# Savasstion/FYPRayTracer

Hardware: AMD Instinct MI355X
Metric: Mrays/s at 1920x1080, 1 spp ReSTIR DI (ms/frame in ms_per_step) (higher is better)
Workload: dtype f32; 1 GPU; hall_1M_tris_256_lights_1920x1080_RESTIR_DI_1spp; triangles=999832, meshes=108, emissive_triangles=256, rays_per_frame=3932782, temporal_reuse=True, spatial_reuse=True, parallelism=row-bands x1

## Files before the change

### fypraytracer_amd/csrc/fyprt.hip

```cpp
#include <hip/hip_runtime.h>
#include <atomic>
#include <cmath>
#include <cstdio>
#include <cstring>
#include <functional>
#include <string>
#include <vector>
#include "rt_host.h"
#include <hipcub/hipcub.hpp>
#include "rt_lbvh.h"
#include "rt_refit.h"
#include "rt_materials.h"
#include "rt_paths.h"
#include "rt_query.h"
#include "rt_points.h"
#include "rt_boxes.h"
#include "rt_denoise.h"
#include "rt_temporal.h"
#include "rt_upscale.h"
#include "rt_probe.h"

using namespace rt;

#ifndef RT_DN_LDS_MAX_STEP
// ... 1459 lines not shown
    const uint32_t tilesX = (c->W + 15u) / 16u, tilesY = (rowEnd - rowBegin + 15u) / 16u;
    return dim3(c->tuning[K_TILE_ORDER] == 2 ? tilesX * ((tilesY + 7u) / 8u) * 8u : ((tilesX * tilesY + 7u) / 8u) * 8u);
}
static unsigned long long* frame_counters(const fyprt_context* c, int part) { return c->countRays ? c->rayCounter.p + 8 * part : nullptr; }
static int check_frame(fyprt_context* c, const fyprt_settings* s, int phase) {
    if (c->hostOnly) return c->fail(FYPRT_ESTATE, "host-only context (device -1) cannot render");
    if (!c->haveScene || !c->haveCamera || c->W == 0) return c->fail(FYPRT_ESTATE, "fyprt_render: resize, upload_scene and set_camera must precede render");
    if (c->dcam.W != c->W || c->dcam.H != c->H) return c->fail(FYPRT_ESTATE, "fyprt_render: camera viewport differs from the render size");
    const int tech = s->technique; const bool restir = tech == FYPRT_RESTIR_DI || tech == FYPRT_RESTIR_GI;
    if (tech < 0 || tech > 8) return c->fail(FYPRT_EINVAL, "fyprt_render: unknown technique");
    if (phase != 0 && !restir) return c->fail(FYPRT_EINVAL, "fyprt_render_part: only the ReSTIR techniques have two parts");
    if (phase == 2 && !c->part1Pending) return c->fail(FYPRT_ESTATE, "fyprt_render_part(2) without a preceding part 1");
    if (phase != 2 && c->part1Pending) return c->fail(FYPRT_ESTATE, "a frame's part 1 is pending: call fyprt_render_part(ctx, settings, 2) first");
    if ((tech == FYPRT_LIGHT_SOURCE_SAMPLING || tech == FYPRT_NEE) && (c->dsc.emissiveCount == 0 || c->dsc.ltTlasCount == 0))
        return c->fail(FYPRT_ENOLIGHT, "fyprt_render: technique needs emissive triangles and a light tree");
    if (tech == FYPRT_RESTIR_DI && c->dsc.emissiveCount == 0) return c->fail(FYPRT_ENOLIGHT, "fyprt_render: ReSTIR DI needs emissive triangles");
    if (restir && stripes_set(c)) return c->fail(FYPRT_ESTATE, "ReSTIR frames need contiguous rows: clear fyprt_set_row_stripes first");
    return FYPRT_OK;
}
static int begin_frame(FrameRun& f) {
    fyprt_context* c = f.c; DevFrame& fr = f.fr;
    HIPCHK(c, hipSetDevice(c->device));
    f.st = dev_settings(c, f.s);
    fr.accum = c->accum.p; fr.image = c->externalImage ? c->externalImage : c->image.p; fr.payload = c->payload.p; fr.depth = c->depth.p;
    fr.normalPrev = c->normalFlip ? c->normalB.p : c->normalA.p; fr.normalCur = c->normalFlip ? c->normalA.p : c->normalB.p;
    fr.di = c->di.p; fr.diPrev = c->diPrev.p; fr.gi = c->gi.p; fr.giPrev = c->giPrev.p; fr.giHot = c->giHot.p;
    fr.drec = c->drec.p; fr.dprevRead = c->dprevFlip ? c->dprevB.p : c->dprevA.p; fr.dprevWrite = c->dprevFlip ? c->dprevA.p : c->dprevB.p;
    fr.W = c->W; fr.H = c->H; fr.frameIndex = c->frameIndex; fr.rowBegin = c->rowBegin; fr.rowEnd = c->rowEnd;
    fr.stripeRows = 0; fr.stripeParts = 1; fr.stripePart = 0; f.striped = stripes_set(c);
    fr.histBegin = (f.tech == FYPRT_RESTIR_GI) ? c->histGI[0] : c->histDI[0]; fr.histEnd = (f.tech == FYPRT_RESTIR_GI) ? c->histGI[1] : c->histDI[1];
#ifdef RT_TOPCACHE
    const uint32_t topCount = (uint32_t)std::min<size_t>((size_t)std::max(0, c->tuning[K_TOP_NODES]), c->hostBvh.nodes.size());
#else
    const uint32_t topCount = 0u;
#endif
    const StackLds stack = stack_lds(c, topCount);
    f.sc = secondary_scene(c->dsc, (uint32_t)c->tuning[K_QUORUM_PRIMARY], frame_counters(c, 0));
    f.sc.stackBudget = stack.budget; f.sc.topCount = topCount; f.ldsBytes = stack.bytes;
    f.par = (int)(c->frameSerial & 1ull); f.wavefront = f.tech == FYPRT_RESTIR_DI && c->tuning[K_DI_WAVEFRONT] == 1;
    f.overlap = f.wavefront && c->tuning[K_PIPELINE] != 0 && !c->countRays && f.phase == 0;
    f.fs = f.overlap ? c->front : c->stream;
    f.split = f.overlap && c->tuning[K_DI_SPLIT] != 0 && !c->blockingCall;
    if (f.overlap) {
        HIPCHK(c, hipStreamWaitEvent(c->front, c->evDone[f.par], 0));
        if (!c->lastOverlapped) HIPCHK(c, hipStreamWaitEvent(c->front, c->evDone[f.par ^ 1], 0));
    }
    if (f.split) HIPCHK(c, hipStreamWaitEvent(c->prim, c->evTemp[f.par], 0));
    c->frameComplete = false;
    if (f.tech != FYPRT_RESTIR_DI) c->drop_kept_primary();
    fr.tileOrder = (uint32_t)c->tuning[K_TILE_ORDER]; fr.p1Mode = f.wavefront ? 1u : 0u;
    f.grid = tile_grid(c, c->rowBegin, c->rowEnd); f.ev = c->ring[c->frameSerial % fyprt_context::kRing];
    if (f.phase == 2) { f.ei = 2; return FYPRT_OK; }
    std::memcpy(c->framePV, c->camPV, 64);
    c->frameCam = c->dcam; c->frameSky = f.st.sky;
    if (c->countRays) HIPCHK(c, hipMemsetAsync(c->rayCounter.p, 0, 256, c->stream));
    if (c->frameIndex == 1) HIPCHK(c, hipMemsetAsync(c->accum.p, 0, c->accum.bytes(), c->stream));
    if (f.timed) HIPCHK(c, hipEventRecord(f.ev[f.ei++], f.split ? c->prim.h : f.fs));
    return FYPRT_OK;
}
static int run_frame_stage(FrameRun& f, const StageRun& r) {
    fyprt_context* c = f.c;
    const StageBufs wf{{c->wfRays[0].p, c->wfRays[1].p}, {c->wfHits[0].p, c->wfHits[1].p}, c->wfState.p, c->wfPixels.p, c->wfPixels2.p, frame_counters(c, 0)};
    return run_stage(c, r, wf, f.sc, c->dcam, f.fr, f.st, f.ldsBytes, c->blockingCall, &f.stageLaunches);
}
static int enqueue_path_frame(FrameRun& f) {
    fyprt_context* c = f.c; DevFrame& fr = f.fr; const int tech = f.tech;
    const PathShape p = path_shape(tech, f.st);
    dim3 pgrid = f.grid;
    if (f.striped) {
        fr.stripeRows = c->stripeRows; fr.stripeParts = c->stripeParts; fr.stripePart = c->stripePart;
        fr.rowBegin = 0; fr.rowEnd = stripe_row_count(c->H, c->stripeRows, c->stripeParts, c->stripePart);
        pgrid = tile_grid(c, fr.rowBegin, fr.rowEnd);
    }
    const size_t entries = (size_t)(fr.rowEnd - fr.rowBegin) * c->W;
    TRY(ensure_paths(c, entries, p.raysPer, p.stride, 3 * p.L));
    HIPCHK(c, hipMemsetAsync(c->wfCounters.p, 0, 3 * p.L * sizeof(uint32_t), c->stream));
    f.launches = 1;
    const bool fused = tech != FYPRT_NEE && (c->tuning[K_FUSED_FRAME] == 2 || (c->tuning[K_FUSED_FRAME] == 0 && c->hostBvh.tris.size() < 65536u));
    if (fused) {
        PathIO io{};
        io.fusedOwner = kNotFused; io.raysIn = c->wfRays[0].p; io.raysOut = c->wfRays[0].p; io.hitsIn = c->wfHits[0].p; io.state = c->wfState.p; io.stateStride = p.stride; io.raysPer = 1u;
        static void (*const kFused[2][6])(DevScene, DevCamera, DevFrame, DevSettings, PathIO, uint32_t) = {{k_path_fused<T_BRUTE, false>, k_path_fused<T_UNIFORM, false>, k_path_fused<T_COSINE, false>, k_path_fused<T_GGX, false>, k_path_fused<T_BRDF, false>, k_path_fused<T_LIGHT, false>},
                                                    {k_path_fused<T_BRUTE, true>, k_path_fused<T_UNIFORM, true>, k_path_fused<T_COSINE, true>, k_path_fused<T_GGX, true>, k_path_fused<T_BRDF, true>, k_path_fused<T_LIGHT, true>}};
        hipLaunchKernelGGL(kFused[c->countRays ? 1 : 0][tech], pgrid, dim3(kBlock), f.ldsBytes, c->stream, f.sc, c->dcam, fr, f.st, io, p.steps);
        return FYPRT_OK;
    }
    hipLaunchKernelGGL(c->countRays ? k_primary<true> : k_primary<false>, pgrid, dim3(kBlock), f.ldsBytes, c->stream, f.sc, c->dcam, fr, f.st, c->wfPixels.p, c->wfCounters.p);
    return run_frame_stage(f, path_stage(tech, p, c->wfPixels.p, c->wfPixels2.p, c->wfCounters.p, entries));
}
struct Part1Rows { uint32_t begin, end, extraRow; size_t pixels; dim3 grid; };
static Part1Rows part1_rows(const fyprt_context* c) {
    const uint32_t halo = (c->haloExchange || c->tuning[K_SKIP_HALO_PART1]) ? 0u : c->halo;
    const uint32_t b = (c->rowBegin > halo) ? c->rowBegin - halo : 0u, e = (c->rowEnd + halo < c->H) ? c->rowEnd + halo : c->H;
    const bool extra = halo > 0 && c->rowBegin < halo && e < c->H;
    return {b, e, extra ? c->H - 1u : 0xFFFFFFFFu, ((size_t)(e - b) + (extra ? 1u : 0u)) * c->W, tile_grid(c, b, extra ? e + 16u : e)};
}
static int enqueue_gi_frame(FrameRun& f) {
    fyprt_context* c = f.c; const Part1Rows p1 = part1_rows(c);
    const uint32_t steps1 = f.st.maxBounces, steps2 = f.st.useSpatial ? f.st.numNeighbors : 0u;
    const size_t L1 = (size_t)steps1 + 2, L2 = (size_t)steps2 + 2;
    TRY(ensure_paths(c, p1.pixels, 1, 5, 2 * L1 + 2 * L2));
    uint32_t* cnt1 = c->wfCounters.p; uint32_t* cnt2 = cnt1 + 2 * L1;
    if (f.phase != 2) {
        TRY(sync_restir_normals(c, f.tech, c->stream));
        HIPCHK(c, hipMemsetAsync(cnt1, 0, (2 * L1 + 2 * L2) * sizeof(uint32_t), c->stream));
        hipLaunchKernelGGL(c->countRays ? k_gi_primary<true> : k_gi_primary<false>, p1.grid, dim3(kBlock), f.ldsBytes, c->stream, f.sc, c->dcam, f.fr, f.st, p1.begin, p1.end, p1.extraRow, c->wfPixels.p, cnt1);
        TRY(run_frame_stage(f, StageRun{T_GI1, steps1, 1u, 5u, c->wfPixels.p, cnt1, cnt1 + L1, c->wfPixels2.p, cnt2, 0, nullptr, p1.pixels}));
        if (f.timed) HIPCHK(c, hipEventRecord(f.ev[f.ei++], c->stream));
        if (f.phase == 1) { f.part1Only = true; return c->hip(hipGetLastError(), "ReSTIR GI part 1"); }
    }
    const DevScene tsc = secondary_scene(f.sc, (uint32_t)c->tuning[K_QUORUM_SECONDARY], frame_counters(c, 1));
    if (c->tuning[K_GI2_MODE] == 2) {
        const int occ = c->gi2Occ.get(k_gi2_persistent<false>, f.ldsBytes, 3), perCU = c->tuning[K_WG_PER_CU] > 0 ? std::min(c->tuning[K_WG_PER_CU], occ) : occ;
        GI2Queue gq{c->wfPixels2.p, cnt2, cnt2 + L2 + 1};
        set_queue_params(c, gq, K_GI2_REFILL_LANES);
        hipLaunchKernelGGL(c->countRays ? k_gi2_persistent<true> : k_gi2_persistent<false>, dim3((uint32_t)(c->numCUs * perCU)), dim3(kBlock), f.ldsBytes, c->stream, tsc, c->dcam, f.fr, f.st, gq);
    } else if (c->tuning[K_GI2_MODE] == 1) {
        const uint32_t fg = (uint32_t)std::max<size_t>(1, std::min<size_t>((size_t)c->numCUs * 64u, (p1.pixels + kBlock - 1) / kBlock));
        hipLaunchKernelGGL(c->countRays ? k_gi2_fused<true> : k_gi2_fused<false>, dim3(fg), dim3(kBlock), f.ldsBytes, c->stream, tsc, c->dcam, f.fr, f.st, (const uint32_t*)c->wfPixels2.p, (const uint32_t*)cnt2);
    } else TRY(run_frame_stage(f, StageRun{T_GI2, steps2, 1u, 5u, c->wfPixels2.p, cnt2, cnt2 + L2, nullptr, nullptr, 1, nullptr, p1.pixels}));
    f.launches = 2; c->normalFlip = !c->normalFlip; c->histGI[0] = c->rowBegin; c->histGI[1] = c->rowEnd;
    return FYPRT_OK;
}
static int enqueue_di_wavefront_part2(FrameRun& f) {
    fyprt_context* c = f.c; const int par = f.par; const dim3 grid = f.grid; hipStream_t fs = f.fs;
    const dim3 block(kBlock);
    ShadowQueue q{};
    q.tasks = c->shadowTasks.p + (size_t)par * c->queueStride; q.rayless = q.tasks + c->queueStride; q.counters = c->queueCounters.p + 4 * par;
    set_queue_params(c, q, K_REFILL_LANES);
    const size_t sg = (size_t)par * c->sortGroups;
    q.sortMode = c->tuning[K_SORT_TASKS] ? 1u : 0u; q.numGroups = grid.x; q.counts = c->sortCounts.p + 2 * sg; q.bases = q.counts + c->sortGroups; q.keys = c->sortKeys.p + sg * 256u; q.hist = c->sortHist.p + sg * kSortBins;
    q.binOffset = c->sortOffset.p + sg * kSortBins; q.binTotal = c->sortTotal.p + (size_t)par * kSortBins; q.sorted = c->sortIndex.p + sg * 256u;
    HIPCHK(c, hipMemsetAsync(q.counters, 0, 16, fs));
    static void (*const kSetup[3])(DevScene, DevCamera, DevFrame, DevSettings, ShadowQueue) = {k_di_part2_setup<0>, k_di_part2_setup<1>, k_di_part2_setup<2>};
    hipLaunchKernelGGL(kSetup[c->tuning[K_SETUP_FETCH]], grid, block, 0, fs, f.sc, c->dcam, f.fr, f.st, q);
    if (q.sortMode) {
        hipLaunchKernelGGL(k_di_sort_scan, dim3(kSortBins), block, 0, fs, q);
        hipLaunchKernelGGL(k_di_sort_scatter, grid, block, 0, fs, q);
    }
    if (f.timed) HIPCHK(c, hipEventRecord(f.ev[f.ei++], fs));
    if (f.overlap) {
        HIPCHK(c, hipEventRecord(c->evFront[par], c->front));
        HIPCHK(c, hipStreamWaitEvent(c->stream, c->evFront[par], 0));
        if (f.timed) HIPCHK(c, hipEventRecord(f.ev[4], c->stream));
    }
    f.sc.rayCounter = frame_counters(c, 2);
    int perCU = c->tuning[K_WG_PER_CU];
    if (perCU <= 0) {
        perCU = c->traceOcc.get(k_di_part2_trace<false>, f.ldsBytes, 4);
        if (f.overlap && perCU > 4) perCU = 4;
    }
    const uint32_t traceGrid = std::max(8u, std::min((uint32_t)(c->numCUs * perCU), grid.x));
    hipLaunchKernelGGL(c->countRays ? k_di_part2_trace<true> : k_di_part2_trace<false>, dim3(traceGrid), block, f.ldsBytes, c->stream, f.sc, f.fr, q);
    f.launches = 3;
    return FYPRT_OK;
}
static bool kept_primary_usable(const fyprt_context* c, const Part1Rows& p1) {
    const fyprt_context::KeptPrimary& k = c->kept; const DevCamera& d = c->dcam;
    return k.valid && !c->countRays && c->tuning[K_KEEP_PRIMARY] != 0 && k.begin == p1.begin && k.end == p1.end && k.extraRow == p1.extraRow && k.rowBegin == c->rowBegin && k.rowEnd == c->rowEnd && k.W == d.W && k.H == d.H &&
           !std::memcmp(&k.invProj, &d.invProj, sizeof d.invProj) && !std::memcmp(&k.invView, &d.invView, sizeof d.invView) && !std::memcmp(&k.position, &d.position, sizeof d.position);
}
static int establish_kept_primary(fyprt_context* c, const Part1Rows& p1, hipStream_t writer) {
    fyprt_context::KeptPrimary& k = c->kept; const DevCamera& d = c->dcam;
    k.valid = true; k.begin = p1.begin; k.end = p1.end; k.extraRow = p1.extraRow; k.rowBegin = c->rowBegin; k.rowEnd = c->rowEnd; k.invProj = d.invProj; k.invView = d.invView; k.position = d.position; k.W = d.W; k.H = d.H; k.writer = writer;
    HIPCHK(c, hipEventRecord(c->evPayload, writer));
    return FYPRT_OK;
}
static int enqueue_di_frame(FrameRun& f) {
    fyprt_context* c = f.c;
    if (f.phase != 2) {
        const Part1Rows p1 = part1_rows(c);
        const bool kept = kept_primary_usable(c, p1);
        if (kept) c->keptFrames++;
        if (f.split) {
            const size_t npx = (size_t)c->W * c->H;
            const DIStage sg{kept ? nullptr : c->stagePayload.p + (size_t)f.par * npx, c->stageRec.p + (size_t)f.par * npx};
            if (kept) {
                HIPCHK(c, hipStreamWaitEvent(c->prim, c->evPayload, 0));
                hipLaunchKernelGGL((k_di_part1_primary<false, true>), p1.grid, dim3(kBlock), 0, c->prim, f.sc, c->dcam, f.fr, f.st, p1.begin, p1.end, p1.extraRow, sg);
            } else hipLaunchKernelGGL((k_di_part1_primary<false, false>), p1.grid, dim3(kBlock), f.ldsBytes, c->prim, f.sc, c->dcam, f.fr, f.st, p1.begin, p1.end, p1.extraRow, sg);
            if (f.timed) HIPCHK(c, hipEventRecord(f.ev[f.ei++], c->prim));
            HIPCHK(c, hipEventRecord(c->evPrim[f.par], c->prim));
            HIPCHK(c, hipStreamWaitEvent(c->front, c->evPrim[f.par], 0));
            TRY(sync_restir_normals(c, f.tech, f.fs));
            if (f.timed) HIPCHK(c, hipEventRecord(f.ev[5], c->front));
            if (kept && c->kept.writer != c->front.h) HIPCHK(c, hipStreamWaitEvent(c->front, c->evPayload, 0));
            hipLaunchKernelGGL(kept ? k_di_part1_temporal<true> : k_di_part1_temporal<false>, p1.grid, dim3(kBlock), 0, c->front, f.sc, c->dcam, f.fr, f.st, p1.begin, p1.end, p1.extraRow, sg);
            HIPCHK(c, hipEventRecord(c->evTemp[f.par], c->front));
            if (!kept) TRY(establish_kept_primary(c, p1, c->front));
        } else {
            TRY(sync_restir_normals(c, f.tech, f.fs));
            if (kept) {
                if (c->kept.writer != f.fs) HIPCHK(c, hipStreamWaitEvent(f.fs, c->evPayload, 0));
                hipLaunchKernelGGL((k_di_part1<false, true>), p1.grid, dim3(kBlock), 0, f.fs, f.sc, c->dcam, f.fr, f.st, p1.begin, p1.end, p1.extraRow);
            } else {
                for (int k = 0; k < 2; ++k) HIPCHK(c, hipStreamWaitEvent(f.fs, c->evPrim[k], 0));
                hipLaunchKernelGGL((c->countRays ? k_di_part1<true, false> : k_di_part1<false, false>), p1.grid, dim3(kBlock), f.ldsBytes, f.fs, f.sc, c->dcam, f.fr, f.st, p1.begin, p1.end, p1.extraRow);
                TRY(establish_kept_primary(c, p1, f.fs));
            }
            if (f.timed) HIPCHK(c, hipEventRecord(f.ev[f.ei++], f.fs));
        }
        if (f.phase == 1) { f.part1Only = true; return c->hip(hipGetLastError(), "ReSTIR DI part 1"); }
    }
    f.sc = secondary_scene(f.sc, (uint32_t)c->tuning[K_QUORUM_SECONDARY], frame_counters(c, 1)); f.launches = 2;
    if (f.wavefront) TRY(enqueue_di_wavefront_part2(f));
    else hipLaunchKernelGGL(c->countRays ? k_di_part2<true> : k_di_part2<false>, f.grid, dim3(kBlock), f.ldsBytes, c->stream, f.sc, c->dcam, f.fr, f.st);
    c->dprevFlip = !c->dprevFlip; c->histDI[0] = c->rowBegin; c->histDI[1] = c->rowEnd;
    return FYPRT_OK;
}
static int end_frame(FrameRun& f) {
    fyprt_context* c = f.c; const unsigned long long slot = c->frameSerial % fyprt_context::kRing;
    HIPCHK(c, hipGetLastError());
    c->part1Pending = false;
    if (f.timed) HIPCHK(c, hipEventRecord(f.ev[f.ei++], c->stream));
    HIPCHK(c, hipEventRecord(c->evDone[f.par], c->stream));
    c->lastOverlapped = f.overlap; c->lastLaunches = f.launches; c->lastTech = f.tech;
    if (f.tech == FYPRT_RESTIR_DI || f.tech == FYPRT_RESTIR_GI) c->lastRestir = f.tech;
    c->ringLaunches[slot] = f.timed ? f.launches : 0; c->ringSplit[slot] = f.split ? 2 : f.overlap ? 1 : 0;
    c->frameSerial++; c->frameComplete = true; c->lastFrameIndex = c->frameIndex;
    if (f.s->to_accumulate) c->frameIndex++; else c->frameIndex = 1;
    return FYPRT_OK;
}
static int enqueue_frame(fyprt_context* c, const fyprt_settings* s, bool timed, int phase = 0) {
    FrameRun f{}; f.c = c; f.s = s; f.tech = s->technique; f.phase = phase; f.timed = timed;
    int rc = check_frame(c, s, phase);
    if (rc == FYPRT_OK) rc = begin_frame(f);
    if (rc == FYPRT_OK) rc = f.tech == FYPRT_RESTIR_DI ? enqueue_di_frame(f) : f.tech == FYPRT_RESTIR_GI ? enqueue_gi_frame(f) : enqueue_path_frame(f);
    if (rc == FYPRT_OK) { if (f.part1Only) c->part1Pending = true; else rc = end_frame(f); }
    if (rc != FYPRT_OK && rc != FYPRT_ESTATE) c->part1Pending = false;
    return rc;
}
static hipError_t part_elapsed(fyprt_context* c, unsigned long long slot, int k, float* ms) {
    const int mode = c->ringSplit[slot], start = (mode && k == 2) ? 4 : (mode == 2 && k == 1) ? 5 : k;
    return hipEventElapsedTime(ms, c->ring[slot][start], c->ring[slot][k + 1]);
}

int fyprt_render(fyprt_context* c, const fyprt_settings* s, fyprt_frame_stats* stats) {
    if (!c || !s) return FYPRT_EINVAL;
    c->blockingCall = true;
    int rc = enqueue_frame(c, s, true);
    c->blockingCall = false;
    if (rc != FYPRT_OK) return rc;
    HIPCHK(c, sync_all(c));
    if (stats) {
        std::memset(stats, 0, sizeof *stats);
        stats->launches = (uint32_t)c->lastLaunches;
        float total = 0.0f;
        for (int k = 0; k < c->lastLaunches; ++k) {
            float ms = 0.0f; (void)part_elapsed(c, (c->frameSerial - 1ull) % fyprt_context::kRing, k, &ms);
            stats->kernel_ms_part[k] = ms; total += ms;
        }
        stats->kernel_ms = total;
        if (c->countRays) {
            unsigned long long r[32] = {0}; (void)hipMemcpy(r, c->rayCounter.p, 256, hipMemcpyDeviceToHost);
            for (int k = 0; k < 4; ++k) add_ray_stats(stats, k, r + 8 * k);
        }
    }
    return FYPRT_OK;
}

int fyprt_render_async(fyprt_context* c, const fyprt_settings* s) { if (!c || !s) return FYPRT_EINVAL; return enqueue_frame(c, s, true); }

int fyprt_frame_timings(fyprt_context* c, uint32_t frames_back, float* kernel_ms_part4, uint32_t* launches) {
    if (!c || !kernel_ms_part4) return FYPRT_EINVAL;
    if (frames_back >= (uint32_t)fyprt_context::kRing || frames_back >= c->frameSerial) return c->fail(FYPRT_EINVAL, "fyprt_frame_timings: frame no longer in the ring");
    const unsigned long long slot = (c->frameSerial - 1ull - frames_back) % fyprt_context::kRing;
    const int n = c->ringLaunches[slot];
    for (int k = 0; k < 4; ++k) kernel_ms_part4[k] = 0.0f;
    for (int k = 0; k < n && k < 4; ++k) {
        float ms = 0.0f;
        const hipError_t e = part_elapsed(c, slot, k, &ms);
        if (e != hipSuccess) return c->hip(e, "hipEventElapsedTime (synchronize the context first)");
        kernel_ms_part4[k] = ms;
    }
    if (launches) *launches = (uint32_t)n;
    return FYPRT_OK;
}
int fyprt_synchronize(fyprt_context* c) { if (!c) return FYPRT_EINVAL; if (c->hostOnly) return FYPRT_OK; HIPCHK(c, hipSetDevice(c->device)); HIPCHK(c, sync_all(c)); return FYPRT_OK; }

int fyprt_readback(fyprt_context* c, uint32_t* rgba8, float* accum4) {
    if (!c) return FYPRT_EINVAL;
    if (c->hostOnly || c->W == 0) return c->fail(FYPRT_ESTATE, "fyprt_readback before fyprt_resize");
    HIPCHK(c, hipSetDevice(c->device));
    HIPCHK(c, sync_all(c));
    const size_t off = (size_t)c->rowBegin * c->W, cnt = (size_t)(c->rowEnd - c->rowBegin) * c->W;
    const uint32_t* img = c->externalImage ? c->externalImage : c->image.p;
    if (rgba8) HIPCHK(c, hipMemcpy(rgba8 + off, img + off, cnt * 4, hipMemcpyDeviceToHost));
    if (accum4) HIPCHK(c, hipMemcpy(accum4 + off * 4, c->accum.p + off, cnt * 16, hipMemcpyDeviceToHost));
    return FYPRT_OK;
}

int fyprt_selftest_math(fyprt_context* c, uint64_t* mismatches3, uint32_t* first_bad3) {
    if (!c || !mismatches3) return FYPRT_EINVAL;
    if (c->hostOnly) return c->fail(FYPRT_ESTATE, "fyprt_selftest_math needs a device");
    HIPCHK(c, hipSetDevice(c->device)); HIPCHK(c, sync_all(c));
    DevBuf<unsigned long long> counts; DevBuf<uint32_t> first;
    HIPCHK(c, counts.alloc(3)); HIPCHK(c, first.alloc(3));
    hipError_t e = hipMemsetAsync(counts.p, 0, 24, c->stream);
    if (e == hipSuccess) e = hipMemsetAsync(first.p, 0xFF, 12, c->stream);
    for (int w = 0; w < 3 && e == hipSuccess; ++w) { hipLaunchKernelGGL(k_math_selftest, dim3((uint32_t)c->numCUs * 16u), dim3(256), 0, c->stream, w, counts.p, first.p); e = hipGetLastError(); }
    unsigned long long hc[3] = {0, 0, 0}; uint32_t hf[3] = {0, 0, 0};
    if (e == hipSuccess) e = hipMemcpyAsync(hc, counts.p, 24, hipMemcpyDeviceToHost, c->stream);
    if (e == hipSuccess) e = hipMemcpyAsync(hf, first.p, 12, hipMemcpyDeviceToHost, c->stream);
    if (e == hipSuccess) e = hipStreamSynchronize(c->stream);
    HIPCHK(c, e);
    for (int w = 0; w < 3; ++w) { mismatches3[w] = hc[w]; if (first_bad3) first_bad3[w] = hf[w]; }
// ... 843 lines not shown
```

### fypraytracer_amd/csrc/rt_wavefront.h

```cpp
#pragma once
#include "rt_kernels.h"

namespace rt {

struct ShadowQueue {
    float4* tasks; uint32_t* counters; uint32_t chunk, refillLanes, staticChunks, minChunk;
    float4* rayless;
    uint32_t sortMode, numGroups; uint32_t* counts; uint32_t* bases; uint8_t* keys; uint16_t* hist; uint32_t* binOffset; uint32_t* binTotal; uint32_t* sorted;
};
constexpr uint32_t kNoRayTask = 0xFFFFFFFFu;
constexpr uint32_t kSortBins = 64;
constexpr int kRefillLanes = 16;

constexpr int kSpecNeighbors = 5;
RT_DEV uint32_t neighbor_from_states(const DevCamera& cam, uint32_t W, uint32_t x, uint32_t y, uint32_t radius, uint32_t s1, uint32_t s2) {
    float ox = 2.0f * ((float)s1 * 0x1p-32f) - 1.0f, oy = 2.0f * ((float)s2 * 0x1p-32f) - 1.0f;
    ox = (float)(uint32_t)(x + (uint32_t)(int)(ox * (float)radius));
    oy = (float)(uint32_t)(y + (uint32_t)(int)(oy * (float)radius));
    ox = __builtin_fmaxf(0.0f, __builtin_fminf((float)cam.W - 1.0f, ox));
    oy = __builtin_fmaxf(0.0f, __builtin_fminf((float)cam.H - 1.0f, oy));
    return (uint32_t)ox + (uint32_t)oy * W;
}
RT_DEV uint32_t spatial_reuse_speculative(const DevCamera& cam, const DevFrame& fr, const DevSettings& st, uint32_t x, uint32_t y, const Payload& pp, uint32_t seed, DIRes& S, uint32_t& Z) {
    const uint32_t N = st.numNeighbors;
// ... 74 lines not shown
    bool live = false, noRay = false;
    f3 ro = splat3(0.0f), rd = splat3(0.0f), Lvis = splat3(0.0f), Lsky = splat3(0.0f); uint32_t ti = kNoRayTask, lightSlot = 0; float tLight = -1.0f;
    Payload pp; Mat hm;
    if (inside) {
        pp = fr.payload[i];
        if (pp.hitDistance < 0.0f) { noRay = true; Lvis = st.sky; }
        else {
            hm = load_mat(sc, tri_material(sc, pp.objectIndex));
            if (length(emission(hm)) > 0.0f) { noRay = true; Lvis = emission(hm); } else live = true;
        }
    }
    if (live) {
        uint32_t seed = i * (fr.frameIndex + 213u + st.randSeed);
        const DIRec own = load_rec(fr.drec + i);
        DIRes R = rec_reservoir(own);
        const f3 pd = ray_direction(cam, x, y);
        if (st.useSpatial) {
            uint32_t Z = 0; DIRes S = di_empty();
            { const float pdf = R.pdf; di_update(S, R.index, (pdf * R.W) * (float)R.M, R.M, pdf, seed); Z += pdf > 0.0f ? R.M : 0u; }
            if (SPECULATIVE && st.numNeighbors <= (uint32_t)kSpecNeighbors) seed = spatial_reuse_speculative(cam, fr, st, x, y, pp, seed, S, Z);
            else if (MODE == 2 && ww != 0u) for (uint32_t n = 0; n < st.numNeighbors; ++n) {
                const uint32_t ni = neighbor_index(cam, fr.W, x, y, st.radius, seed);
                const uint32_t nxp = ni % fr.W, nyp = ni / fr.W;
                float nd; f2 nn;
                if (nxp - wx0 < ww && nyp - wy0 < wh) { const uint32_t k = (nyp - wy0) * ww + (nxp - wx0); nd = s_win[k]; nn.x = s_win[kWinMax * kWinMax + k]; nn.y = s_win[2 * kWinMax * kWinMax + k]; }
                else { const float4 h = reinterpret_cast<const float4*>(fr.drec + ni)[0]; nd = h.x; nn.x = h.y; nn.y = h.z; }
                const float pdp = pp.hitDistance;
                if ((nd > 1.1f * pdp || nd < 0.9f * pdp) || (double)dot(nrm3(pp), oct_decode(nn)) < 0.906) continue;
                const DIRes N = rec_reservoir(load_rec(fr.drec + ni));
                const float pdf = N.pdf;
                di_update(S, N.index, (pdf * N.W) * (float)N.M, N.M, pdf, seed);
                Z += pdf > 0.0f ? N.M : 0u;
            }
            else for (uint32_t n = 0; n < st.numNeighbors; ++n) {
                const uint32_t ni = neighbor_index(cam, fr.W, x, y, st.radius, seed);
                const DIRec nb = load_rec(fr.drec + ni);
                const float nd = nb.hitDistance, pdp = pp.hitDistance;
                f2 nn; nn.x = nb.nx; nn.y = nb.ny;
                const DIRes N = rec_reservoir(nb);
                if ((nd > 1.1f * pdp || nd < 0.9f * pdp) || (double)dot(nrm3(pp), oct_decode(nn)) < 0.906) continue;
                const float pdf = N.pdf;
                di_update(S, N.index, (pdf * N.W) * (float)N.M, N.M, pdf, seed);
                Z += pdf > 0.0f ? N.M : 0u;
            }
            const float m = 1.0f / (float)Z;
            S.W = S.pdf > 0.0f ? (1.0f / S.pdf) * (m * S.wSum) : 0.0f;
            R = S;
        }
        lightSlot = R.index;
        const float4* LR = sc.lightRecs + (size_t)R.index * 3;
        const float4 l0 = LR[0], l1 = LR[1], l2 = LR[2];
        ti = (uint32_t)__float_as_int(l1.w);
        const TriGeom g = load_tri(sc, ti);
        const f3 ep = tri_random_point(g, seed);
        f3 dir = ep - pos3(pp);
        const float dist = length(pos3(pp) - ep);
        dir = dir / dist;
        const f3 albedo = sample_albedo(sc, hm, pp.u, pp.v);
        const f3 brdf = eval_brdf(nrm3(pp), -pd, dir, albedo, hm.metallic, hm.roughness);
        const float cx = gmax(dot(dir, nrm3(pp)), 0.0f);
        const float cy = gmax(dot(-dir, mk3(l1.x, l1.y, l1.z)), 0.0f);
        const float sa = l0.w * (dist * dist);
        const f3 T = ((brdf * cx) * cy) / sa;
        const f3 lem = mk3(l2.x, l2.y, l2.z);
        if (length(lem) > 0.0f) { Lvis = T * lem; Lvis = Lvis * R.W; }
        Lsky = T * st.sky;
        ro = pos3(pp) + nrm3(pp) * 1e-12f; rd = dir;
        if (st.skipDeadRays && zero3(Lvis) && zero3(Lsky)) ti = kNoRayTask;
        else tLight = light_tri_distance(sc, ti, ro, rd);
        fr.depth[i] = pp.hitDistance;
        { f2 on; on.x = own.nx; on.y = own.ny; store_rec(fr.dprevWrite + i, pp.hitDistance, on, R); }
    }
    __shared__ uint32_t s_count[kBlock / 64];
    __shared__ unsigned long long s_base;
    __shared__ uint32_t s_hist[kSortBins];
    const bool hasRay = live && ti != kNoRayTask, rayless = (live || noRay) && !hasRay;
    const unsigned long long mask = __ballot(hasRay), emptyMask = __ballot(rayless);
    const uint32_t lane = threadIdx.x & 63u, wave = threadIdx.x >> 6;
    if (lane == 0u) s_count[wave] = (uint32_t)__popcll(mask) | ((uint32_t)__popcll(emptyMask) << 16);
    if (q.sortMode && threadIdx.x < kSortBins) s_hist[threadIdx.x] = 0u;
    __syncthreads();
    const uint32_t nBoth = s_count[0] + s_count[1] + s_count[2] + s_count[3], nRays = nBoth & 0xFFFFu, nEmpty = nBoth >> 16;
    const unsigned long long below = (1ull << lane) - 1ull;
    uint32_t rank = (uint32_t)__popcll(mask & below) | ((uint32_t)__popcll(emptyMask & below) << 16);
    for (uint32_t k = 0; k < wave; ++k) rank += s_count[k];
    if (threadIdx.x == 0u) s_base = nBoth ? atomicAdd(reinterpret_cast<unsigned long long*>(q.counters), (unsigned long long)nRays | ((unsigned long long)nEmpty << 32)) : 0ull;
    __syncthreads();
    const uint32_t slot = (uint32_t)s_base + (rank & 0xFFFFu);
    if (q.sortMode) {
        const uint32_t key = (uint32_t)(((unsigned long long)lightSlot * kSortBins) / (sc.emissiveCount ? sc.emissiveCount : 1u));
        if (hasRay) { atomicAdd(&s_hist[key], 1u); q.keys[slot] = (uint8_t)key; }
        __syncthreads();
        if (threadIdx.x < kSortBins) q.hist[(size_t)blockIdx.x * kSortBins + threadIdx.x] = (uint16_t)s_hist[threadIdx.x];
        if (threadIdx.x == 0u) { q.counts[blockIdx.x] = nRays; q.bases[blockIdx.x] = (uint32_t)s_base; }
    }
    if (hasRay) {
        float4* t = q.tasks + (size_t)slot * 4;
        t[0] = make_float4(ro.x, ro.y, ro.z, tLight);
        t[1] = make_float4(rd.x, rd.y, rd.z, __int_as_float((int)ti));
        t[2] = make_float4(Lvis.x, Lvis.y, Lvis.z, __int_as_float((int)i));
        t[3] = make_float4(Lsky.x, Lsky.y, Lsky.z, __int_as_float((int)i));
    } else if (rayless) {
        const size_t k = (size_t)(uint32_t)(s_base >> 32) + (rank >> 16);
        q.rayless[-1 - (ptrdiff_t)k] = make_float4(Lvis.x, Lvis.y, Lvis.z, __int_as_float((int)i));
    }
}

__global__ __launch_bounds__(kBlock) void k_di_sort_scan(ShadowQueue q) {
    __shared__ uint32_t s_part[kBlock];
    const uint32_t bin = blockIdx.x, t = threadIdx.x;
    const uint32_t per = (q.numGroups + kBlock - 1u) / kBlock, g0 = t * per, g1 = (g0 + per < q.numGroups) ? g0 + per : q.numGroups;
    uint32_t sum = 0;
    for (uint32_t g = g0; g < g1; ++g) sum += q.hist[(size_t)g * kSortBins + bin];
    s_part[t] = sum;
    __syncthreads();
    for (uint32_t d = 1; d < (uint32_t)kBlock; d <<= 1) {
        const uint32_t add = (t >= d) ? s_part[t - d] : 0u;
        __syncthreads();
        s_part[t] += add;
        __syncthreads();
    }
    uint32_t run = s_part[t] - sum;
    for (uint32_t g = g0; g < g1; ++g) { q.binOffset[(size_t)g * kSortBins + bin] = run; run += q.hist[(size_t)g * kSortBins + bin]; }
    if (t == (uint32_t)kBlock - 1u) q.binTotal[bin] = s_part[t];
}
__global__ __launch_bounds__(kBlock) void k_di_sort_scatter(ShadowQueue q) {
    __shared__ uint32_t s_start[kSortBins];
    __shared__ uint32_t s_rank[kSortBins];
    const uint32_t g = blockIdx.x, t = threadIdx.x;
    if (t < kSortBins) s_rank[t] = 0u;
    if (t == 0u) {
        uint32_t run = 0;
        for (uint32_t b = 0; b < kSortBins; ++b) { s_start[b] = run; run += q.binTotal[b]; }
    }
    __syncthreads();
    if (t < q.counts[g]) {
        const uint32_t slot = q.bases[g] + t, key = q.keys[slot];
        const uint32_t r = atomicAdd(&s_rank[key], 1u);
        q.sorted[s_start[key] + q.binOffset[(size_t)g * kSortBins + key] + r] = slot;
    }
}

struct LaneRay {
    f3 o, d; RayPk pk; float tL, cut; uint32_t lightTri, task;
    int32_t cur; int top; int32_t hitTri; bool closestMode; uint32_t nBox, nTri, nNode;
};

RT_DEV void lane_push(int32_t* lds, int& top, int32_t v) { lds[top * kBlock] = v; ++top; }
RT_DEV int32_t lane_pop(int32_t* lds, int& top) { --top; return lds[top * kBlock]; }

#ifndef RT_TRACE_WAVES
#define RT_TRACE_WAVES __attribute__((amdgpu_waves_per_eu(6)))
#endif
template <bool COUNT>
RT_DEV void di_part2_trace_body(const DevScene& sc, const DevFrame& fr, const ShadowQueue& q, int32_t* s_stack) {
    int32_t* lds = s_stack + threadIdx.x;
    const float4* top4 = stage_top_nodes(sc.nodes, sc.topCount, sc.stackBudget, s_stack);
    const uint32_t lane = threadIdx.x & 63u;
    const uint32_t total = q.counters[0];
    const uint32_t nWaves = gridDim.x * (uint32_t)(kBlock / 64), myWave = blockIdx.x * (uint32_t)(kBlock / 64) + (threadIdx.x >> 6);
    const uint32_t share = (total + nWaves - 1u) / nWaves;
    const uint32_t chunk = q.chunk;
    const uint32_t want1 = chunk * q.staticChunks;
    const uint32_t first = share < want1 ? (share < 16u ? 16u : share) : want1;
    const uint32_t dynBase = nWaves * first;
    const bool hasDyn = dynBase < total;
    for (uint32_t k = myWave * 64u + lane, nEmpty = q.counters[1]; k < nEmpty; k += nWaves * 64u) {
        const float4 L = q.rayless[-1 - (ptrdiff_t)k];
        epilogue(fr, (uint32_t)__float_as_int(L.w), rgb1(mk3(L.x, L.y, L.z)));
    }
    LaneRay r; r.cur = kExit; r.top = 0; r.nBox = 0; r.nTri = 0; r.nNode = 0;
    bool active = false;
    bool pending = false;
    uint32_t outcome = 0;
    bool more = total != 0u;
    uint32_t chunkNext = myWave * first < total ? myWave * first : total;
    uint32_t chunkEnd = (myWave + 1u) * first < total ? (myWave + 1u) * first : total;
    while (true) {
        const unsigned long long idle = __ballot(!active);
        if ((more && (uint32_t)__popcll(idle) >= q.refillLanes) || __ballot(active) == 0ull) {
            if (pending) {
                const float4 L = q.tasks[(size_t)r.task * 4 + (outcome == 2u ? 3 : 2)];
                const uint32_t pixel = (uint32_t)__float_as_int(L.w);
                const f3 radiance = (outcome != 0u) ? mk3(L.x, L.y, L.z) : splat3(0.0f);
                epilogue(fr, pixel, rgb1(radiance)); pending = false;
            }
        }
        if (more && (uint32_t)__popcll(idle) >= q.refillLanes) {
            if (chunkNext >= chunkEnd && hasDyn) {
                uint32_t base = 0;
                uint32_t size = (total - chunkEnd) / nWaves;
                size = size < q.minChunk ? q.minChunk : (size > chunk ? chunk : size);
                if (lane == 0u) base = dynBase + atomicAdd(q.counters + 2, size);
                base = (uint32_t)__shfl((int)base, 0);
                chunkNext = base < total ? base : total;
                chunkEnd = (base + size < total) ? base + size : total;
            }
            const uint32_t slot = chunkNext + (uint32_t)__popcll(idle & ((1ull << lane) - 1ull));
            const uint32_t want = (uint32_t)__popcll(idle), avail = chunkEnd - chunkNext;
            chunkNext += (want < avail) ? want : avail;
            more = chunkNext < chunkEnd || (hasDyn && chunkEnd < total);
            if (!active && slot < chunkEnd) {
                r.task = q.sortMode ? q.sorted[slot] : slot;
                const float4* t = q.tasks + (size_t)r.task * 4;
                const float4 t0 = t[0], t1 = t[1];
                r.o = mk3(t0.x, t0.y, t0.z);
                r.d = mk3(t1.x, t1.y, t1.z); r.lightTri = (uint32_t)__float_as_int(t1.w);
                r.pk = make_raypk(r.o, safe_inv(r.d.x), safe_inv(r.d.y), safe_inv(r.d.z));
                const float tL = t0.w;
                r.closestMode = !(tL > 0.0f);
                r.tL = r.closestMode ? 3.402823466e+38f : tL;
                r.cut = r.tL * 1.000001f;
                r.hitTri = r.closestMode ? -1 : (int32_t)r.lightTri;
                if (COUNT) { r.nBox = 0; r.nTri = 1; r.nNode = 0; }
                r.top = 0; lane_push(lds, r.top, kExit);
                r.cur = (sc.triCount == 0 || ray_not_finite(r.o, r.d)) ? kExit : sc.rootRef;
                active = true;
            }
        }
        if (__ballot(active) == 0ull) { if (!more) break; else continue; }
        while (true) {
            bool walk = active && r.cur >= 0;
            const uint32_t quorum = quorum_of(sc.nodeQuorum, (uint32_t)__popcll(__ballot(active)));
            while (walk) {
                { Stack st; st.lds = lds; st.top = r.top; st.top4 = top4; st.topCount = sc.topCount; r.cur = node_step<COUNT>(sc.nodes, sc.stackBudget, r.cur, r.pk, r.cut, st, r.nBox, r.nNode); r.top = st.top; }
                walk = r.cur >= 0;
                if ((uint32_t)__popcll(__ballot(walk)) < quorum) break;
            }
            if (active && r.cur < 0 && r.cur != kExit) {
                const uint32_t code = (uint32_t)~r.cur, first = code >> 2, cnt = (code & 3u) + 1u;
                bool occluded = false;
                for (uint32_t k = 0; k < cnt; ++k) {
                    const float4* tp = sc.leafTris + (size_t)(first + k) * 3;
                    const float4 a = tp[0], b = tp[1], c = tp[2];
                    const uint32_t id = (uint32_t)__float_as_int(c.y);
                    if (!r.closestMode && id == r.lightTri) continue;
                    if (COUNT) r.nTri += 1;
                    const f3 v0 = mk3(a.x, a.y, a.z), e1 = mk3(a.w, b.x, b.y), e2 = mk3(b.z, b.w, c.x);
                    const f3 hh = cross(r.d, e2);
                    const float det = dot(e1, hh), f = 1.0f / det;
                    const f3 s = r.o - v0;
                    const float u = f * dot(s, hh);
                    if (u < 0.0f || u > 1.0f) continue;
                    const f3 qq = cross(s, e1);
                    const float v = f * dot(r.d, qq);
                    if (v < 0.0f || (u + v) > 1.0f) continue;
                    const float t = f * dot(e2, qq);
                    if (t > 0.0001f && t < r.tL) {
                        r.hitTri = (int32_t)id;
                        if (r.closestMode) { r.tL = t; r.cut = t * 1.000001f; }
                        else { occluded = true; break; }
                    }
                }
                r.cur = occluded ? kExit : lane_pop(lds, r.top);
            }
            if (active && r.cur == kExit) {
                outcome = 0u;
                if (r.hitTri == (int32_t)r.lightTri) outcome = 1u;
                else if (r.closestMode && r.hitTri < 0) outcome = 2u;
                pending = true;
                if (COUNT) {
                    atomicAdd(sc.rayCounter + 0, 1ull); atomicAdd(sc.rayCounter + 1, (unsigned long long)r.nBox);
                    atomicAdd(sc.rayCounter + 2, (unsigned long long)r.nTri);
                    atomicAdd(sc.rayCounter + 3, (unsigned long long)((r.closestMode && r.hitTri < 0) ? 0 : 1));
                    atomicAdd(sc.rayCounter + 4, (unsigned long long)r.nNode);
                }
                active = false;
            }
            const unsigned long long act = __ballot(active);
            if (act == 0ull) break;
            if (more && (64u - (uint32_t)__popcll(act)) >= q.refillLanes) break;
        }
    }
}

template <bool COUNT> __global__ void k_di_part2_trace(DevScene sc, DevFrame fr, ShadowQueue q);
template <> __global__ __launch_bounds__(kBlock) RT_TRACE_WAVES void k_di_part2_trace<false>(DevScene sc, DevFrame fr, ShadowQueue q) {
    extern __shared__ int32_t s_stack[];
    di_part2_trace_body<false>(sc, fr, q, s_stack);
}
template <> __global__ __launch_bounds__(kBlock) void k_di_part2_trace<true>(DevScene sc, DevFrame fr, ShadowQueue q) {
    extern __shared__ int32_t s_stack[];
    di_part2_trace_body<true>(sc, fr, q, s_stack);
}

constexpr uint32_t kRayClosest = 0xFFFFFFFEu, kRayVisible = 0xFFFFFFFDu;
constexpr uint32_t kRayNone = 0xFFFFFFFCu;
struct TraceQueue {
    const float4* rays; float4* hits; const uint32_t* count; uint32_t raysPer; uint32_t* head;
    uint32_t chunk, refillLanes, staticChunks, minChunk;
};

template <bool COUNT>
RT_DEV void trace_rays_body(const DevScene& sc, const TraceQueue& q, int32_t* s_stack) {
    int32_t* lds = s_stack + threadIdx.x;
    const uint32_t lane = threadIdx.x & 63u;
    const uint32_t total = *q.count * q.raysPer;
    const uint32_t nWaves = gridDim.x * (uint32_t)(kBlock / 64), myWave = blockIdx.x * (uint32_t)(kBlock / 64) + (threadIdx.x >> 6);
    const uint32_t share = (total + nWaves - 1u) / nWaves;
    const uint32_t chunk = q.chunk, want1 = chunk * q.staticChunks;
    const uint32_t first = share < want1 ? (share < 16u ? 16u : share) : want1;
    const uint32_t dynBase = nWaves * first;
    const bool hasDyn = dynBase < total;
    f3 o = splat3(0.0f), d = splat3(0.0f); RayPk pk = make_raypk(o, 1.0f, 1.0f, 1.0f);
    float tL = 0.0f, cut = 0.0f, hu = 0.0f, hv = 0.0f; uint32_t mode = kRayClosest, task = 0; int32_t cur = kExit, hitTri = -1; int top = 0;
    bool closestMode = true;
    uint32_t nBox = 0, nTri = 0, nNode = 0;
    bool active = false;
    bool more = total != 0u;
    uint32_t chunkNext = myWave * first < total ? myWave * first : total;
    uint32_t chunkEnd = (myWave + 1u) * first < total ? (myWave + 1u) * first : total;
    while (true) {
        const unsigned long long idle = __ballot(!active);
        if (more && (uint32_t)__popcll(idle) >= q.refillLanes) {
            if (chunkNext >= chunkEnd && hasDyn) {
                uint32_t base = 0;
                uint32_t size = (total - chunkEnd) / nWaves;
                size = size < q.minChunk ? q.minChunk : (size > chunk ? chunk : size);
                if (lane == 0u) base = dynBase + atomicAdd(q.head, size);
                base = (uint32_t)__shfl((int)base, 0);
                chunkNext = base < total ? base : total;
                chunkEnd = (base + size < total) ? base + size : total;
            }
            const uint32_t slot = chunkNext + (uint32_t)__popcll(idle & ((1ull << lane) - 1ull));
            const uint32_t want = (uint32_t)__popcll(idle), avail = chunkEnd - chunkNext;
            chunkNext += (want < avail) ? want : avail;
            more = chunkNext < chunkEnd || (hasDyn && chunkEnd < total);
            if (!active && slot < chunkEnd) {
                task = slot;
                const float4* t = q.rays + (size_t)task * 3;
                const float4 t0 = t[0], t1 = t[1], t2 = t[2];
                o = mk3(t0.x, t0.y, t0.z); d = mk3(t1.x, t1.y, t1.z); mode = (uint32_t)__float_as_int(t1.w);
                pk = make_raypk(o, safe_inv(d.x), safe_inv(d.y), safe_inv(d.z));
                hitTri = -1; hu = 0.0f; hv = 0.0f; closestMode = true; tL = 3.402823466e+38f;
                if (mode == kRayVisible) { closestMode = false; hu = t2.x - t2.y; tL = t2.x + t2.y; }
                else if (mode != kRayClosest && t2.x > 0.0f) { closestMode = false; tL = t2.x; hitTri = (int32_t)mode; }
                cut = tL * 1.000001f;
                if (COUNT) { nBox = 0; nNode = 0; nTri = (mode != kRayClosest && mode != kRayVisible) ? 1u : 0u; }
                top = 0; lane_push(lds, top, kExit);
                cur = (sc.triCount == 0 || mode == kRayNone || ray_not_finite(o, d)) ? kExit : sc.rootRef;
                active = true;
            }
        }
        if (__ballot(active) == 0ull) { if (!more) break; else continue; }
        while (true) {
            bool walk = active && cur >= 0;
            const uint32_t quorum = quorum_of(sc.nodeQuorum, (uint32_t)__popcll(__ballot(active)));
            while (walk) {
                { Stack st; st.lds = lds; st.top = top; cur = node_step<COUNT>(sc.nodes, sc.stackBudget, cur, pk, cut, st, nBox, nNode); top = st.top; }
                walk = cur >= 0;
                if ((uint32_t)__popcll(__ballot(walk)) < quorum) break;
            }
            if (active && cur < 0 && cur != kExit) {
                const uint32_t code = (uint32_t)~cur, firstTri = code >> 2, cnt = (code & 3u) + 1u;
                bool done = false;
                for (uint32_t k = 0; k < cnt; ++k) {
                    const float4* tp = sc.leafTris + (size_t)(firstTri + k) * 3;
                    if (!closestMode && (uint32_t)__float_as_int(tp[2].y) == mode) continue;
                    float t, u, v; uint32_t id;
                    if (COUNT) nTri += 1;
                    if (!tri_test(tp, o, d, t, u, v, id)) continue;
                    if (mode == kRayVisible) {
                        if (t < hu) { hv = -1.0f; done = true; break; }
                        if (t <= tL) hv = 1.0f;
                    } else if (t < tL) {
                        hitTri = (int32_t)id; tL = t;
                        if (closestMode) { cut = t * 1.000001f; hu = u; hv = v; }
                        else { done = true; break; }
                    }
                }
                cur = done ? kExit : lane_pop(lds, top);
            }
            if (active && cur == kExit) {
                float4 res;
                if (mode == kRayVisible) res = make_float4(hv > 0.0f ? 1.0f : 0.0f, 0.0f, 0.0f, 0.0f);
                else res = make_float4(hitTri < 0 ? -1.0f : tL, hu, hv, __int_as_float(hitTri));
                q.hits[task] = res;
                if (COUNT && mode != kRayNone) {
                    atomicAdd(sc.rayCounter + 0, 1ull); atomicAdd(sc.rayCounter + 1, (unsigned long long)nBox);
                    atomicAdd(sc.rayCounter + 2, (unsigned long long)nTri);
                    atomicAdd(sc.rayCounter + 3, (unsigned long long)((mode == kRayVisible) ? (hv > 0.0f ? 1 : 0) : (hitTri < 0 ? 0 : 1)));
                    atomicAdd(sc.rayCounter + 4, (unsigned long long)nNode);
                }
                active = false;
            }
            const unsigned long long act = __ballot(active);
            if (act == 0ull) break;
            if (more && (64u - (uint32_t)__popcll(act)) >= q.refillLanes) break;
        }
    }
}

template <bool COUNT>
RT_DEV float4 trace_one(const DevScene& sc, f3 o, f3 d, uint32_t mode, float a0, float a1, int32_t* ldsBase) {
    float tL = 3.402823466e+38f, hu = 0.0f, hv = 0.0f; int32_t hitTri = -1; bool closestMode = true;
    if (mode == kRayVisible) { closestMode = false; hu = a0 - a1; tL = a0 + a1; }
    else if (mode != kRayClosest && a0 > 0.0f) { closestMode = false; tL = a0; hitTri = (int32_t)mode; }
    float cut = tL * 1.000001f;
    uint32_t nBox = 0, nNode = 0, nTri = (mode != kRayClosest && mode != kRayVisible) ? 1u : 0u;
    if (!(sc.triCount == 0 || ray_not_finite(o, d))) {
        const RayPk pk = make_raypk(o, safe_inv(d.x), safe_inv(d.y), safe_inv(d.z));
        Stack st; st.lds = ldsBase; st.top = 0; st.push(kExit);
        int32_t cur = sc.rootRef;
        bool done = false;
        while (!done) {
            bool walk = cur >= 0;
            const uint32_t quorum = quorum_of(sc.nodeQuorum, (uint32_t)__popcll(__ballot(true)));
            while (walk) {
                cur = node_step<COUNT>(sc.nodes, sc.stackBudget, cur, pk, cut, st, nBox, nNode);
                walk = cur >= 0;
                if ((uint32_t)__popcll(__ballot(walk)) < quorum) break;
            }
// ... 56 lines not shown
```

Before: 6224 Mrays/s.

## Test shadow-ray leaf triangles cooperatively across wave lanes

When any lane of a wave reaches a multi-triangle leaf and no lane is in closest-hit mode, the (ray, triangle) pairs of all lanes are packed into LDS so that each lane tests one pair. Ray data is fetched from the owning lane with ds_bpermute and occlusion is gathered back with a ballot. This is meant to cut divergent serial leaf loops, at the cost of extra ballots, LDS writes, wave barriers and permutes on every leaf step. The change also moves outcome computation to the point of use and swaps a shfl/popcount for readfirstlane/mbcnt.

```diff
diff --git a/fypraytracer_amd/csrc/fyprt.hip b/fypraytracer_amd/csrc/fyprt.hip
--- a/fypraytracer_amd/csrc/fyprt.hip
+++ b/fypraytracer_amd/csrc/fyprt.hip
@@ -1635,6 +1635,14 @@
     }
     const uint32_t traceGrid = std::max(8u, std::min((uint32_t)(c->numCUs * perCU), grid.x));
     hipLaunchKernelGGL(c->countRays ? k_di_part2_trace<true> : k_di_part2_trace<false>, dim3(traceGrid), block, f.ldsBytes, c->stream, f.sc, f.fr, q);
+#ifdef RT_DI_LEAF_STATS
+    {
+        uint32_t kinds = 0;
+        HIPCHK(c, hipStreamSynchronize(c->stream));
+        HIPCHK(c, hipMemcpy(&kinds, q.counters + 3, sizeof kinds, hipMemcpyDeviceToHost));
+        std::fprintf(stderr, "fyprt leaf phases: grid %u, rays %s, kinds 0x%x (1 one round, 2 over 64 pairs, 4 single-triangle leaves, 8 closest-mode lane)\n", traceGrid, c->countRays ? "counted" : "production", kinds);
+    }
+#endif
     f.launches = 3;
     return FYPRT_OK;
 }
diff --git a/fypraytracer_amd/csrc/rt_wavefront.h b/fypraytracer_amd/csrc/rt_wavefront.h
--- a/fypraytracer_amd/csrc/rt_wavefront.h
+++ b/fypraytracer_amd/csrc/rt_wavefront.h
@@ -250,8 +250,32 @@
 #ifndef RT_TRACE_WAVES
 #define RT_TRACE_WAVES __attribute__((amdgpu_waves_per_eu(6)))
 #endif
+#ifndef RT_DI_COOP_LEAF
+#define RT_DI_COOP_LEAF 1
+#endif
+
+RT_DEV bool leaf_tri_test(const float4 a, const float4 b, const float4 c, const f3 o, const f3 d, float& t) {
+    const f3 v0 = mk3(a.x, a.y, a.z), e1 = mk3(a.w, b.x, b.y), e2 = mk3(b.z, b.w, c.x);
+    const f3 hh = cross(d, e2);
+    const float det = dot(e1, hh), f = 1.0f / det;
+    const f3 s = o - v0;
+    const float u = f * dot(s, hh);
+    if (u < 0.0f || u > 1.0f) return false;
+    const f3 qq = cross(s, e1);
+    const float v = f * dot(d, qq);
+    if (v < 0.0f || (u + v) > 1.0f) return false;
+    t = f * dot(e2, qq);
+    return true;
+}
+RT_DEV uint32_t lanes_below(unsigned long long mask) { return __builtin_amdgcn_mbcnt_hi((uint32_t)(mask >> 32), __builtin_amdgcn_mbcnt_lo((uint32_t)mask, 0u)); }
+RT_DEV void wave_lds_order() { __builtin_amdgcn_fence(__ATOMIC_RELEASE, "wavefront"); __builtin_amdgcn_wave_barrier(); __builtin_amdgcn_fence(__ATOMIC_ACQUIRE, "wavefront"); }
+RT_DEV float lane_read(int byteLane, float v) { return __int_as_float(__builtin_amdgcn_ds_bpermute(byteLane, __float_as_int(v))); }
+
 template <bool COUNT>
 RT_DEV void di_part2_trace_body(const DevScene& sc, const DevFrame& fr, const ShadowQueue& q, int32_t* s_stack) {
+    constexpr bool COOP = !COUNT && RT_DI_COOP_LEAF != 0;
+    uint8_t* pairs = nullptr;
+    if constexpr (COOP) { __shared__ uint8_t s_pairs[kBlock]; pairs = s_pairs + (uint32_t)__builtin_amdgcn_readfirstlane((int)(threadIdx.x >> 6)) * 64u; }
     int32_t* lds = s_stack + threadIdx.x;
     const float4* top4 = stage_top_nodes(sc.nodes, sc.topCount, sc.stackBudget, s_stack);
     const uint32_t lane = threadIdx.x & 63u;
@@ -270,7 +294,7 @@
     LaneRay r; r.cur = kExit; r.top = 0; r.nBox = 0; r.nTri = 0; r.nNode = 0;
     bool active = false;
     bool pending = false;
-    uint32_t outcome = 0;
+    auto outcome_of = [](const LaneRay& x) -> uint32_t { return x.hitTri == (int32_t)x.lightTri ? 1u : (x.closestMode && x.hitTri < 0) ? 2u : 0u; };
     bool more = total != 0u;
     uint32_t chunkNext = myWave * first < total ? myWave * first : total;
     uint32_t chunkEnd = (myWave + 1u) * first < total ? (myWave + 1u) * first : total;
@@ -278,6 +302,7 @@
         const unsigned long long idle = __ballot(!active);
         if ((more && (uint32_t)__popcll(idle) >= q.refillLanes) || __ballot(active) == 0ull) {
             if (pending) {
+                const uint32_t outcome = outcome_of(r);
                 const float4 L = q.tasks[(size_t)r.task * 4 + (outcome == 2u ? 3 : 2)];
                 const uint32_t pixel = (uint32_t)__float_as_int(L.w);
                 const f3 radiance = (outcome != 0u) ? mk3(L.x, L.y, L.z) : splat3(0.0f);
@@ -290,11 +315,11 @@
                 uint32_t size = (total - chunkEnd) / nWaves;
                 size = size < q.minChunk ? q.minChunk : (size > chunk ? chunk : size);
                 if (lane == 0u) base = dynBase + atomicAdd(q.counters + 2, size);
-                base = (uint32_t)__shfl((int)base, 0);
+                base = (uint32_t)__builtin_amdgcn_readfirstlane((int)base);
                 chunkNext = base < total ? base : total;
                 chunkEnd = (base + size < total) ? base + size : total;
             }
-            const uint32_t slot = chunkNext + (uint32_t)__popcll(idle & ((1ull << lane) - 1ull));
+            const uint32_t slot = chunkNext + lanes_below(idle);
             const uint32_t want = (uint32_t)__popcll(idle), avail = chunkEnd - chunkNext;
             chunkNext += (want < avail) ? want : avail;
             more = chunkNext < chunkEnd || (hasDyn && chunkEnd < total);
@@ -325,7 +350,52 @@
                 walk = r.cur >= 0;
                 if ((uint32_t)__popcll(__ballot(walk)) < quorum) break;
             }
-            if (active && r.cur < 0 && r.cur != kExit) {
+            const bool atLeaf = active && r.cur < 0 && r.cur != kExit;
+            bool serialLeaves = true;
+            if constexpr (COOP) {
+                const uint32_t cnt = atLeaf ? ((uint32_t)~r.cur & 3u) + 1u : 0u;
+                const unsigned long long m1 = __ballot(atLeaf), m2 = __ballot(cnt >= 2u);
+                serialLeaves = m2 == 0ull || __ballot(atLeaf && r.closestMode) != 0ull;
+#ifdef RT_DI_LEAF_STATS
+                {
+                    const uint32_t n = (uint32_t)(__popcll(m1) + __popcll(m2) + __popcll(__ballot(cnt >= 3u)) + __popcll(__ballot(cnt >= 4u)));
+                    if (m1 != 0ull && lane == 0u) atomicOr(q.counters + 3, m2 == 0ull ? 4u : serialLeaves ? 8u : n > 64u ? 2u : 1u);
+                }
+#endif
+                if (!serialLeaves) {
+                    const unsigned long long m3 = __ballot(cnt >= 3u), m4 = __ballot(cnt >= 4u);
+                    const uint32_t prefix = lanes_below(m1) + lanes_below(m2) + lanes_below(m3) + lanes_below(m4);
+                    const uint32_t nPairs = (uint32_t)(__popcll(m1) + __popcll(m2) + __popcll(m3) + __popcll(m4));
+                    bool occluded = false;
+                    for (uint32_t base = 0; base < nPairs; base += 64u) {
+#pragma unroll
+                        for (uint32_t k = 0; k < 4u; ++k)
+                            if (k < cnt && prefix + k - base < 64u) __hip_atomic_store(pairs + (prefix + k - base), (uint8_t)(lane | (k << 6)), __ATOMIC_RELAXED, __HIP_MEMORY_SCOPE_WAVEFRONT);
+                        wave_lds_order();
+                        const uint32_t word = __hip_atomic_load(pairs + lane, __ATOMIC_RELAXED, __HIP_MEMORY_SCOPE_WAVEFRONT);
+                        wave_lds_order();
+                        const bool helps = base + lane < nPairs;
+                        const int own = (int)(word & 63u) << 2;
+                        const uint32_t tri = ((uint32_t)~__builtin_amdgcn_ds_bpermute(own, r.cur) >> 2) + ((word >> 6) & 3u);
+                        const f3 o = mk3(lane_read(own, r.o.x), lane_read(own, r.o.y), lane_read(own, r.o.z));
+                        const f3 d = mk3(lane_read(own, r.d.x), lane_read(own, r.d.y), lane_read(own, r.d.z));
+                        const float tL = lane_read(own, r.tL);
+                        const uint32_t lightTri = (uint32_t)__builtin_amdgcn_ds_bpermute(own, (int)r.lightTri);
+                        bool hit = false;
+                        if (helps) {
+                            const float4* tp = sc.leafTris + (size_t)tri * 3;
+                            const float4 a = tp[0], b = tp[1], c = tp[2];
+                            float t;
+                            hit = (uint32_t)__float_as_int(c.y) != lightTri && leaf_tri_test(a, b, c, o, d, t) && t > 0.0001f && t < tL;
+                        }
+                        const unsigned long long hits = __ballot(hit);
+                        const int lo = (int)prefix - (int)base, hi = lo + (int)cnt, lo0 = lo < 0 ? 0 : lo, hi0 = hi > 64 ? 64 : hi;
+                        if (hi0 > lo0) occluded = occluded || ((hits >> lo0) & (~0ull >> (64 - (hi0 - lo0)))) != 0ull;
+                    }
+                    if (atLeaf) { if (occluded) r.hitTri = -1; r.cur = occluded ? kExit : lane_pop(lds, r.top); }
+                }
+            }
+            if (serialLeaves && atLeaf) {
                 const uint32_t code = (uint32_t)~r.cur, first = code >> 2, cnt = (code & 3u) + 1u;
                 bool occluded = false;
                 for (uint32_t k = 0; k < cnt; ++k) {
@@ -353,9 +423,6 @@
                 r.cur = occluded ? kExit : lane_pop(lds, r.top);
             }
             if (active && r.cur == kExit) {
-                outcome = 0u;
-                if (r.hitTri == (int32_t)r.lightTri) outcome = 1u;
-                else if (r.closestMode && r.hitTri < 0) outcome = 2u;
                 pending = true;
                 if (COUNT) {
                     atomicAdd(sc.rayCounter + 0, 1ull); atomicAdd(sc.rayCounter + 1, (unsigned long long)r.nBox);
```

Result: faster. 6421 Mrays/s (median of 6 runs) (+3.2%).
